# NVIDIA-Genomics-Research/racon-gpu

Hardware: AMD Instinct MI355X
Metric: Mbp polished/sec (whole node), ONT C.elegans, at 1/2/4/8 MI355X (higher is better)
Workload: dtype int16

## Files before the change

### src/hip/hip_polisher.cpp

```cpp
#include <hip/hip_runtime.h>

#include <atomic>
#include <chrono>
#include <memory>
#include <mutex>
#include <stdexcept>
#include <string>
#include <thread>
#include <tuple>
#include <utility>
#include <vector>

#include "core/polisher.hpp"
#include "hip/aligner_batch.hpp"
#include "hip/hip_common.hpp"
#include "hip/poa_batch.hpp"

namespace rga {

namespace {

struct BatchPools {
  std::mutex mutex;
  std::vector<std::pair<uint64_t, std::unique_ptr<hip::AlignerBatch>>> aligner;
// ... 424 lines not shown
    }
    const auto& bb = layers.front();
    auto w = createWindow(0, 0, tgs ? WindowType::kTGS : WindowType::kNGS,
                          std::get<0>(bb).data(),
                          static_cast<uint32_t>(std::get<0>(bb).size()),
                          std::get<1>(bb).data(),
                          static_cast<uint32_t>(std::get<1>(bb).size()));
    for (size_t i = 1; i < layers.size(); ++i) {
      const auto& l = layers[i];
      const std::string& q = std::get<1>(l);
      w->add_layer(std::get<0>(l).data(), static_cast<uint32_t>(std::get<0>(l).size()),
                   q.empty() ? nullptr : q.data(), static_cast<uint32_t>(q.size()),
                   std::get<2>(l), std::get<3>(l));
    }
    windows.push_back(std::move(w));
  }
  return windows;
}

std::vector<std::pair<std::string, bool>> poa_windows_gpu(
    const std::vector<std::vector<std::tuple<std::string, std::string, uint32_t, uint32_t>>>&
        window_layers,
    int8_t match, int8_t mismatch, int8_t gap, bool banded, bool trim, bool tgs,
    bool large_graphs, bool score_check) {
  std::vector<std::pair<std::string, bool>> out(window_layers.size());
  std::vector<std::shared_ptr<Window>> windows =
      windows_from_layers(window_layers, tgs, "poa_windows_gpu");

  hip::PoaBatch batch(0, 4ull << 30, match, mismatch, gap, banded, 200, large_graphs,
                      score_check);
  size_t begin = 0;
  std::vector<int64_t> slot_of(windows.size(), -1);
  auto flush = [&](size_t end) {
    std::vector<bool> status = batch.generate(trim);
    size_t k = 0;
    for (size_t i = begin; i < end; ++i) {
      if (slot_of[i] >= 0) {
        out[i] = {windows[i]->consensus(), status[k++]};
      }
    }
    batch.reset();
    begin = end;
  };
  size_t next_slot = 0;
  for (size_t i = 0; i < windows.size(); ++i) {
    if (windows[i]->num_layers() < 3) {
      auto bb = windows[i]->sequence(0);
      out[i] = {std::string(bb.first, bb.second), false};
      continue;
    }
    bool never_fits = false;
    if (batch.add_window(windows[i], &never_fits)) {
      slot_of[i] = static_cast<int64_t>(next_slot++);
      continue;
    }
    if (never_fits) {
      out[i] = {std::string(), false};
      continue;
    }
    flush(i);
    next_slot = 0;
    if (batch.add_window(windows[i], &never_fits)) {
      slot_of[i] = static_cast<int64_t>(next_slot++);
    } else {
      out[i] = {std::string(), false};
    }
  }
  flush(windows.size());
  return out;
}

std::vector<std::tuple<int32_t, std::vector<uint16_t>, std::vector<std::vector<uint16_t>>>>
poa_window_graph_gpu(const RawWindows& window_layers, int8_t match, int8_t mismatch, int8_t gap,
                     bool banded, bool large_graphs, bool score_check) {
  std::vector<std::shared_ptr<Window>> windows =
      windows_from_layers(window_layers, true, "poa_window_graph_gpu");
  hip::PoaBatch batch(0, 4ull << 30, match, mismatch, gap, banded, 200, large_graphs,
                      score_check);
  for (const auto& w : windows) {
    bool never_fits = false;
    if (w->num_layers() < 3 || !batch.add_window(w, &never_fits)) {
      throw std::runtime_error(
          "poa_window_graph_gpu: every window must run on the device, in one batch");
    }
  }
  std::vector<std::tuple<int32_t, std::vector<uint16_t>, std::vector<std::vector<uint16_t>>>> out(
      windows.size());
  if (windows.empty()) {
    return out;
  }
  (void)batch.generate(false);
  for (size_t i = 0; i < windows.size(); ++i) {
    const hip::PoaBatch::WindowGraph g = batch.read_graph(static_cast<uint32_t>(i));
    std::vector<std::vector<uint16_t>> edges(g.rank.size());
    for (size_t node = 0; node < edges.size(); ++node) {
      const uint16_t* row = g.out_edges.data() + node * hip::kPoaLimits.max_edges;
      edges[node].assign(row, row + std::min<uint32_t>(g.out_cnt[node], hip::kPoaLimits.max_edges));
    }
    out[i] = {g.status, g.rank, std::move(edges)};
  }
  return out;
// ... 109 lines not shown
```

### src/hip/hip_polisher_stub.cpp

```cpp
#include <cstdio>
#include <cstdlib>
#include <memory>
#include <string>
#include <tuple>
#include <utility>
#include <vector>

#include "core/polisher.hpp"
#include "hip/aligner_types.hpp"
#include "hip/comm.hpp"
#include "hip/poa_types.hpp"

namespace rga {

namespace comm {
Communicator::~Communicator() {}
void Communicator::init(int, int, const std::string&, int, bool) {
  fprintf(stderr, "[rga::comm] error: no HIP backend in this build!\n");
  exit(1);
}
void Communicator::finalize() {}
std::vector<std::string> Communicator::gather(const std::string&, int) { return {}; }
double Communicator::allreduce_max(double v) { return v; }
double Communicator::allreduce_sum(double v) { return v; }
void Communicator::barrier() {}
void Communicator::ctl_send(int, const void*, size_t) {}
void Communicator::ctl_recv(int, void*, size_t) {}
std::vector<std::string> Communicator::ctl_gather(const std::string&, int) { return {}; }
void Communicator::ctl_bcast(void*, size_t, int) {}
Communicator& world_comm() {
  static Communicator c;
  return c;
}
}

namespace hip {
int runtime_device_count() { return 0; }
void runtime_device_synchronize() {}
void release_batch_pools() {}
std::vector<std::pair<std::string, bool>> poa_windows_gpu(
    const std::vector<std::vector<std::tuple<std::string, std::string, uint32_t, uint32_t>>>&,
    int8_t, int8_t, int8_t, bool, bool, bool, bool, bool) {
  fprintf(stderr, "[rga::hip::poa_windows_gpu] error: no HIP backend in this build!\n");
  exit(1);
}
std::vector<std::tuple<int32_t, std::vector<uint16_t>, std::vector<std::vector<uint16_t>>>>
poa_window_graph_gpu(
    const std::vector<std::vector<std::tuple<std::string, std::string, uint32_t, uint32_t>>>&,
    int8_t, int8_t, int8_t, bool, bool, bool) {
  fprintf(stderr, "[rga::hip::poa_window_graph_gpu] error: no HIP backend in this build!\n");
  exit(1);
}
std::vector<std::tuple<std::string, int32_t, int32_t>> align_pairs(
    const std::vector<std::pair<std::string, std::string>>&, uint32_t, AlnBandPolicy,
    bool) {
  fprintf(stderr, "[rga::hip::align_pairs] error: no HIP backend in this build!\n");
  exit(1);
}
std::vector<std::tuple<std::vector<std::pair<uint32_t, uint32_t>>, int32_t, int32_t>>
breaking_points_pairs(const std::vector<std::pair<std::string, std::string>>&, uint32_t,
                      const std::vector<uint32_t>&, const std::vector<uint32_t>&, uint32_t,
                      AlnBandPolicy, bool) {
  fprintf(stderr, "[rga::hip::breaking_points_pairs] error: no HIP backend in this build!\n");
  exit(1);
}
}

std::unique_ptr<Polisher> createHipPolisher(std::unique_ptr<SequenceParser>,
                                            std::unique_ptr<OverlapParser>,
                                            std::unique_ptr<SequenceParser>, PolisherConfig) {
  fprintf(stderr,
          "[racon::createPolisher] error: HIP pipeline requested but this build "
// ... 6 lines not shown
```

### src/hip/poa_batch.cpp

```cpp
#include "hip/poa_batch.hpp"

#include <hip/hip_runtime.h>

#include <algorithm>
#include <chrono>
#include <cstring>
#include <stdexcept>
#include <type_traits>

#include "hip/hip_common.hpp"

namespace rga::hip {

namespace {

constexpr size_t kSeqArenaPerWindow = 96 * 1024;

constexpr PoaLimits L = kPoaLimits;
constexpr PoaLimits LL = kPoaLargeLimits;

constexpr size_t kLargeBudgetDivisor = 4;
constexpr size_t kLargeSlabCap = 2048;
constexpr size_t kLargePerWindow =
    poa_slab_bytes<true>() + LL.max_consensus * 3 + sizeof(PoaWindowDesc) + 1024;
// ... 112 lines not shown
    if (large_slabs_ > 1) {
      large_slabs_ /= 2;
    }
  }

  RGA_HIP_TRY(hipHostMalloc(reinterpret_cast<void**>(&h_seq_), seq_arena_cap_));
  RGA_HIP_TRY(hipHostMalloc(reinterpret_cast<void**>(&h_weight_), seq_arena_cap_));
  RGA_HIP_TRY(hipHostMalloc(reinterpret_cast<void**>(&h_layer_ends_), max_layers * 4));
  RGA_HIP_TRY(hipHostMalloc(reinterpret_cast<void**>(&h_layer_span_), max_layers * 4));
  RGA_HIP_TRY(hipHostMalloc(reinterpret_cast<void**>(&h_layer_index_), (num_slabs_ + 1) * 4));
  RGA_HIP_TRY(hipHostMalloc(reinterpret_cast<void**>(&h_desc_),
                            num_slabs_ * sizeof(PoaWindowDesc)));
  RGA_HIP_TRY(hipHostMalloc(reinterpret_cast<void**>(&h_consensus_),
                            static_cast<size_t>(num_slabs_) * L.max_consensus));
  RGA_HIP_TRY(hipHostMalloc(reinterpret_cast<void**>(&h_coverage_),
                            static_cast<size_t>(num_slabs_) * L.max_consensus * 2));
  RGA_HIP_TRY(hipHostMalloc(reinterpret_cast<void**>(&h_consensus_len_), num_slabs_ * 4));
  RGA_HIP_TRY(hipHostMalloc(reinterpret_cast<void**>(&h_status_), num_slabs_ * 4));

  lay_out(d_pool_);
  arena_.match = match_;
  arena_.mismatch = mismatch_;
  arena_.gap = gap_;
  arena_.band_width = banded ? 256 : 0;

  if (large_slabs_ != 0) {
    allocate_large_pool();
  }
}

void PoaBatch::allocate_large_pool() {
  large_arena_ = arena_;
  auto lay_out = [&](void* base) {
    size_t total = 0;
    auto carve = [&](auto*& p, size_t count) {
      p = reinterpret_cast<std::remove_reference_t<decltype(p)>>(
          reinterpret_cast<uintptr_t>(base) + total);
      total += (count * sizeof(*p) + 255) & ~size_t(255);
    };
    const size_t slabs = large_slabs_;
    carve(large_arena_.layer_ends_index, slabs + 1);
    carve(large_arena_.windows, slabs);
    for_each_poa_slab<true>(large_arena_.slabs,
                            [&](auto*& p, size_t count) { carve(p, slabs * count); });
    carve(large_arena_.timing, slabs * kPoaTimingSlots);
    carve(large_arena_.consensus, slabs * LL.max_consensus);
// ... 190 lines not shown
  std::vector<PoaWindowDesc> desc_sorted(nw0);
  std::vector<uint32_t> lidx_sorted(nw0);
  launch_slot_.assign(nw0, 0);
  for (uint32_t w = 0; w < nw0; ++w) {
    desc_sorted[w] = h_desc_[perm[w]];
    lidx_sorted[w] = h_layer_index_[perm[w]];
    launch_slot_[perm[w]] = w;
  }
  std::copy(desc_sorted.begin(), desc_sorted.end(), h_desc_);
  std::copy(lidx_sorted.begin(), lidx_sorted.end(), h_layer_index_);

  RGA_HIP_CHECK(hipSetDevice(device_));
  auto s = static_cast<hipStream_t>(stream_);
  auto d = [&](const void* dst, const void* src, size_t bytes) {
    RGA_HIP_CHECK(hipMemcpyAsync(const_cast<void*>(dst), src, bytes, hipMemcpyHostToDevice, s));
  };
  d(arena_.seq_data, h_seq_, seq_bytes_);
  d(arena_.weight_data, h_weight_, seq_bytes_);
  d(arena_.layer_ends, h_layer_ends_, num_layer_ends_ * 4);
  d(arena_.layer_spans, h_layer_span_, num_layer_ends_ * 4);
  d(arena_.layer_ends_index, h_layer_index_, windows_.size() * 4);
  d(arena_.windows, h_desc_, windows_.size() * sizeof(PoaWindowDesc));

  for (uint32_t begin = 0, end; begin < nw0; begin = end) {
    const PoaVariant v = variant_of[perm[begin]];
    for (end = begin + 1; end < nw0 && variant_of[perm[end]] == v; ++end) {
    }
    if (score_check_) {
      launch_poa_kernel_checked(arena_, begin, end - begin, v, stream_);
    } else {
      launch_poa_kernel(arena_, begin, end - begin, v, stream_);
    }
  }

  const size_t nw = windows_.size();
  RGA_HIP_CHECK(hipMemcpyAsync(h_consensus_, arena_.consensus,
                               nw * L.max_consensus, hipMemcpyDeviceToHost, s));
  RGA_HIP_CHECK(hipMemcpyAsync(h_coverage_, arena_.coverage,
                               nw * L.max_consensus * 2, hipMemcpyDeviceToHost, s));
  RGA_HIP_CHECK(hipMemcpyAsync(h_consensus_len_, arena_.consensus_len, nw * 4,
                               hipMemcpyDeviceToHost, s));
  RGA_HIP_CHECK(hipMemcpyAsync(h_status_, arena_.status, nw * 4, hipMemcpyDeviceToHost, s));
  auto t1 = clk::now();
  RGA_HIP_CHECK(hipStreamSynchronize(s));
  auto t2 = clk::now();

  large_completed_ = 0;
  large_slab_of_.assign(nw, -1);
  large_nodes_of_.assign(nw, 0);
  auto t_post = t2;
  if (large_slabs_ != 0) {
    const uint32_t ran = run_large_pass();
    t_post = clk::now();
    if (host_timing && ran != 0) {
      fprintf(stderr,
              "[rga::hip::PoaBatch] host timing: large-graph pass over %u window(s) %.1f ms\n",
              ran,
              std::chrono::duration_cast<std::chrono::microseconds>(t_post - t2).count() /
                  1000.0);
    }
  }

  if (getenv("RGA_POA_TIMING") != nullptr) {
    constexpr size_t kSlots = kPoaTimingSlots;
    std::vector<unsigned long long> t(nw * kSlots);
    RGA_HIP_CHECK(hipMemcpy(t.data(), arena_.timing, t.size() * sizeof(t[0]),
                            hipMemcpyDeviceToHost));
    unsigned long long sum[kSlots] = {0};
    std::vector<unsigned long long> totals(nw);
    for (size_t i = 0; i < nw; ++i) {
      for (size_t k = 0; k < kSlots; ++k) sum[k] += t[i * kSlots + k];
      totals[i] = t[i * kSlots + 6];
    }
    std::sort(totals.begin(), totals.end());
    fprintf(stderr,
            "[rga::hip::PoaBatch] timing (wall ticks, %zu windows): dp=%llu tb=%llu "
            "add=%llu topo=%llu rdesc=%llu cons=%llu total=%llu layers=%llu\n"
            "[rga::hip::PoaBatch] window total ticks: p50=%llu p90=%llu p99=%llu max=%llu\n",
            nw, sum[0], sum[1], sum[2], sum[3], sum[4], sum[5], sum[6], sum[7],
            totals[nw / 2], totals[nw * 9 / 10], totals[nw * 99 / 100], totals[nw - 1]);
  }

  score_refused_ = 0;
  for (size_t i = 0; i < nw; ++i) {
    const uint32_t orig = perm[i];
    auto& window = windows_[orig];
    if (h_status_[i] == kPoaScoreRange) {
      ++score_refused_;
    }
    if (h_status_[i] != kPoaOk || h_consensus_len_[i] == 0) {
      polished[orig] = false;
      continue;
    }
    std::string consensus(reinterpret_cast<char*>(h_consensus_ + i * L.max_consensus),
                          h_consensus_len_[i]);
    bool status = true;
    if (window->type() == WindowType::kTGS && trim) {
      const uint16_t* cov = h_coverage_ + i * L.max_consensus;
      uint32_t average = seqs_added_[orig] / 2;
      int32_t begin = 0, end = static_cast<int32_t>(consensus.size()) - 1;
      for (; begin < static_cast<int32_t>(consensus.size()); ++begin) {
        if (cov[begin] >= average) {
// ... 91 lines not shown
    for (uint32_t k = 0; k < n; ++k) {
      const uint32_t slot = todo[begin + k];
      h_status_[slot] = h_large_status_[k];
      h_consensus_len_[slot] = h_large_consensus_len_[k];
      std::memcpy(h_consensus_ + static_cast<size_t>(slot) * L.max_consensus,
                  h_large_consensus_ + static_cast<size_t>(k) * LL.max_consensus,
                  LL.max_consensus);
      std::memcpy(h_coverage_ + static_cast<size_t>(slot) * L.max_consensus,
                  h_large_coverage_ + static_cast<size_t>(k) * LL.max_consensus,
                  LL.max_consensus * 2);
      large_slab_of_[slot] = static_cast<int32_t>(k);
      large_nodes_of_[slot] = h_large_num_nodes_[k];
      large_slab_owner_[k] = slot;
    }

    if (timing) {
      constexpr size_t kSlots = kPoaTimingSlots;
      std::vector<unsigned long long> t(n * kSlots);
      RGA_HIP_CHECK(hipMemcpy(t.data(), large_arena_.timing, t.size() * sizeof(t[0]),
                              hipMemcpyDeviceToHost));
      unsigned long long sum[kSlots] = {0};
      unsigned long long longest = 0;
      for (size_t i = 0; i < n; ++i) {
        for (size_t k = 0; k < kSlots; ++k) sum[k] += t[i * kSlots + k];
        longest = std::max(longest, t[i * kSlots + 6]);
      }
      fprintf(stderr,
              "[rga::hip::PoaBatch] large-graph pass timing (wall ticks, %u windows): dp=%llu "
              "tb=%llu add=%llu topo=%llu rdesc=%llu cons=%llu total=%llu layers=%llu max=%llu\n",
              n, sum[0], sum[1], sum[2], sum[3], sum[4], sum[5], sum[6], sum[7], longest);
    }
  }
  return static_cast<uint32_t>(todo.size());
}

PoaBatch::WindowGraph PoaBatch::read_graph(uint32_t index) const {
  if (index >= launch_slot_.size() || launch_slot_.size() != windows_.size()) {
    throw std::runtime_error("[rga::hip::PoaBatch] read_graph: no such window in the last run");
  }
  RGA_HIP_CHECK(hipSetDevice(device_));
  WindowGraph g;
  g.status = h_status_[launch_slot_[index]];
  if (g.status != kPoaOk) {
    return g;
  }
  uint32_t n = 0;
  const PoaSlabs* slabs = &arena_.slabs;
// ... 20 lines not shown
    slab = static_cast<size_t>(index) * L.max_nodes;
  }
  static_assert(L.max_edges == LL.max_edges);
  g.rank.resize(n);
  g.out_cnt.resize(n);
  g.out_edges.resize(static_cast<size_t>(n) * L.max_edges);
  if (n != 0) {
    RGA_HIP_CHECK(hipMemcpy(g.rank.data(), slabs->rank + slab, n * sizeof(uint16_t),
                            hipMemcpyDeviceToHost));
    RGA_HIP_CHECK(hipMemcpy(g.out_cnt.data(), slabs->out_cnt + slab, n,
                            hipMemcpyDeviceToHost));
    RGA_HIP_CHECK(hipMemcpy(g.out_edges.data(), slabs->out_edges + slab * L.max_edges,
                            g.out_edges.size() * sizeof(uint16_t), hipMemcpyDeviceToHost));
  }
  return g;
}

void PoaBatch::reset() {
  launch_slot_.clear();
  large_slab_of_.clear();
  large_nodes_of_.clear();
  large_completed_ = 0;
  score_refused_ = 0;
  windows_.clear();
  seqs_added_.clear();
  pending_orders_.clear();
  packed_upto_ = 0;
  seq_bytes_ = 0;
  num_layer_ends_ = 0;
}

}
```

### src/hip/poa_batch.hpp

```cpp
#pragma once

#include <cstdint>
#include <memory>
#include <vector>

#include "core/window.hpp"
#include "hip/poa_types.hpp"

namespace rga::hip {

class PoaBatch {
 public:
  PoaBatch(int device, size_t mem_budget, int8_t match, int8_t mismatch, int8_t gap,
           bool banded, uint32_t max_depth, bool large_graphs = false,
           bool score_check = false);
  ~PoaBatch();

  PoaBatch(const PoaBatch&) = delete;
  PoaBatch& operator=(const PoaBatch&) = delete;

  bool add_window(const std::shared_ptr<Window>& window, bool* never_fits);

  void pack();

  uint32_t size() const { return static_cast<uint32_t>(windows_.size()); }
  uint32_t capacity() const { return num_slabs_; }

  static bool large_scores_fit(int8_t match, int8_t mismatch, int8_t gap, bool banded);
  uint32_t large_capacity() const { return large_slabs_; }
  uint32_t large_completed() const { return large_completed_; }

  static bool score_check_applies(int8_t match, int8_t mismatch, int8_t gap, bool banded,
                                  bool score_check);
  bool score_checked() const { return score_check_; }
  uint32_t score_refused() const { return score_refused_; }

  std::vector<bool> generate(bool trim);

  struct WindowGraph {
    int32_t status = kPoaNotRun;
    std::vector<uint16_t> rank;
    std::vector<uint8_t> out_cnt;
    std::vector<uint16_t> out_edges;
  };
  WindowGraph read_graph(uint32_t index) const;

  void reset();

 private:
  void allocate_arenas(bool banded);
  void allocate_large_pool();
  void release_all();
  uint32_t run_large_pass();

  int device_;
  void* stream_ = nullptr;

  uint32_t num_slabs_;
  size_t seq_arena_cap_;
  int8_t match_, mismatch_, gap_;
  uint32_t max_depth_;
  bool score_check_ = false;
  uint32_t score_refused_ = 0;

  uint8_t* h_seq_ = nullptr;
  uint8_t* h_weight_ = nullptr;
  uint32_t* h_layer_ends_ = nullptr;
  uint32_t* h_layer_span_ = nullptr;
  uint32_t* h_layer_index_ = nullptr;
  PoaWindowDesc* h_desc_ = nullptr;
  uint8_t* h_consensus_ = nullptr;
  uint16_t* h_coverage_ = nullptr;
  uint32_t* h_consensus_len_ = nullptr;
  int32_t* h_status_ = nullptr;

  void* d_pool_ = nullptr;
  PoaDeviceArena arena_{};

  size_t seq_bytes_ = 0;
  size_t num_layer_ends_ = 0;
  std::vector<std::shared_ptr<Window>> windows_;
  std::vector<uint32_t> seqs_added_;
  std::vector<std::vector<uint32_t>> pending_orders_;
  size_t packed_upto_ = 0;
  std::vector<uint32_t> launch_slot_;

// ... 18 lines not shown
```

### src/hip/poa_kernel.hip

```cpp
#include <hip/hip_runtime.h>

#include <cstdio>
#include <cstdlib>

#include "hip/poa_types.hpp"

namespace rga::hip {

namespace {

constexpr int kLanes = 64;
constexpr int32_t kNegInf = -(1 << 28);
#ifdef RGA_POA_LARGE_CLASS
constexpr bool kLarge = true;
#else
constexpr bool kLarge = false;
#endif
#ifdef RGA_POA_SCORE_CHECK
constexpr bool kChecked = true;
#else
constexpr bool kChecked = false;
#endif
constexpr PoaLimits kL = poa_limits(kLarge);
constexpr uint32_t kMaxW = kL.matrix_width;
// ... 855 lines not shown
      if (cbase + WB < kMaxW) {
        *reinterpret_cast<uint64_t*>(Mrow + cbase) = mvpack;
      } else {
        for (uint32_t w = 0; w < nown; ++w) {
          Mrow[cbase + w] = static_cast<uint8_t>(mvpack >> (8 * w));
        }
      }
    }
    if (len > base && len <= base + kLanes * WB) {
      const int owner = static_cast<int>((len - 1 - base) / WB);
      last_col_val = __builtin_amdgcn_readlane(h_sel, owner);
    }
  }

  wave_lds_sync();

  if ((is_end || (d.sub && r == d.rhi)) && last_col_val > best_score) {
    best_score = last_col_val;
    best_row = r + 1;
  }
}


constexpr uint32_t kTbDepth = 64;
static_assert(kTbDepth <= kLanes, "one lane per predicted move");

#define RGA_GLOBAL __attribute__((address_space(1)))
struct TracebackArrays {
  RGA_GLOBAL const uint8_t* moves;
  RGA_GLOBAL const uint64_t* row_desc;
  RGA_GLOBAL const uint16_t* rank;
  RGA_GLOBAL const uint16_t* in_edges;
  RGA_GLOBAL int32_t* aln_nodes;
};
using LdsU16 = __attribute__((address_space(3))) uint16_t;

__device__ __attribute__((noinline)) int32_t traceback_d(const TracebackArrays c, LdsU16* pred0,
                                                         uint32_t rlo, uint32_t best_row,
                                                         uint32_t len, int lane) {
  int32_t status = kPoaOk;
  for (uint32_t r = rlo + 1 + lane; r <= best_row; r += kLanes) {
    const uint32_t p = static_cast<uint32_t>((c.row_desc[r - 1] >> 32) & 0xffff);
    pred0[r] = static_cast<uint16_t>(p > rlo ? p : 0);
  }
  __syncthreads();

// ... 87 lines not shown
  static_assert(MAXW <= kMaxW, "ring width exceeds the slab matrix width");
  static_assert(MAXN <= kMaxN, "node cap exceeds the slab graph capacity");
  if (blockIdx.x >= num_windows) {
    return;
  }
  const uint32_t win = window_base + blockIdx.x;
  const int lane = threadIdx.x;
  const PoaWindowDesc desc = a.windows[win];

  __shared__ Shared<MAXW, MAXN> s;

  WindowCtx c;
  static_cast<PoaSlabs&>(c) = a.slabs;
  for_each_poa_slab<kLarge>(c, [slab = static_cast<size_t>(desc.scratch_idx)](auto*& p,
                                                                              size_t count) {
    p += slab * count;
  });

  unsigned long long* timing = a.timing + static_cast<size_t>(win) * kPoaTimingSlots;
  unsigned long long tick = TIMED ? wall_clock64() : 0;
  const unsigned long long t_start = tick;
  unsigned long long t_dp = 0, t_tb = 0, t_add = 0, t_topo = 0, t_rd = 0, t_cons = 0;
  unsigned long long layers_done = 0;
  auto lap = [&]() -> unsigned long long {
    if (!TIMED) {
      return 0;
    }
    unsigned long long now = wall_clock64();
    unsigned long long d = now - tick;
    tick = now;
    return d;
  };

  c.seq_base = a.seq_data + desc.seq_offset;
  c.weight_base = a.weight_data + desc.seq_offset;
  c.ends = a.layer_ends + a.layer_ends_index[win];
  c.spans = a.layer_spans + a.layer_ends_index[win];
  c.num_seqs = desc.num_seqs;
  c.MN = MAXN - 1;
  c.m = a.match;
  c.x = a.mismatch;
  c.g = a.gap;
  c.status = kPoaOk;

  init_backbone_d(c, s, lane);

// ... 7 lines not shown
    }
    if (len + 1 > MAXW) {
      c.status = kPoaWidthOverflow;
      break;
    }

    build_match_bits_d(s, seq, len, lane);

    const uint32_t n = c.num_nodes;
    LayerDp d;
    d.seq = seq;
    d.len = len;
    d.chunks = (len + kLanes - 1) / kLanes;
    const uint32_t span_word = c.spans[layer];
    d.sub = span_word != 0xFFFFFFFFu;
    d.rlo = d.sub ? c.rank[span_word >> 16] : 0;
    d.rhi = d.sub ? c.rank[span_word & 0xffffu] : n - 1;
    d.bw = a.band_width;
    d.banded = !CHECKED && (d.bw != 0) && (d.bw < len);
    d.slope16 = d.banded ? static_cast<uint32_t>((static_cast<uint64_t>(len) << 16) /
                                                 (d.rhi - d.rlo + 1))
                         : 0;

    int32_t best_score = kNegInf;
    uint32_t best_row = 0;
    uint32_t score_low = 0;
    (void)lap();

    for (uint32_t rblk = d.rlo & ~(kLanes - 1); rblk <= d.rhi; rblk += kLanes) {
      if (rblk + lane < n) {
        s.u.dp.rd_block[lane] = c.row_desc[rblk + lane];
        s.u.dp.rd2_block[lane] = c.row_desc2[rblk + lane];
      }
      wave_lds_sync();
      const uint32_t rlim = min(d.rhi + 1, rblk + kLanes);
      for (uint32_t r = max(rblk, d.rlo); r < rlim; ++r) {
        dp_row<CHECKED, WB, MAXW>(c, s, d, r, s.u.dp.rd_block[r - rblk],
                                  s.u.dp.rd2_block[r - rblk], lane, best_score, best_row,
                                  score_low);
      }
      wave_lds_sync();
    }

    t_dp += lap();
    ++layers_done;

    int lane_g = lane;
    asm volatile("" : "+v"(lane_g));

    if (CHECKED && score_low != 0) {
      c.status = kPoaScoreRange;
    }

    if (!CHECKED || c.status == kPoaOk) {
      c.status = traceback_d({(RGA_GLOBAL const uint8_t*)c.moves,
                              (RGA_GLOBAL const uint64_t*)c.row_desc,
                              (RGA_GLOBAL const uint16_t*)c.rank,
                              (RGA_GLOBAL const uint16_t*)c.in_edges,
                              (RGA_GLOBAL int32_t*)c.aln_nodes},
// ... 27 lines not shown
    t_rd += lap();
  }

  if (lane == 0) {
    uint8_t* out = a.consensus + static_cast<size_t>(win) * kL.max_consensus;
    uint16_t* cov = a.coverage + static_cast<size_t>(win) * kL.max_consensus;
    int32_t clen = -1;
    (void)lap();
    if (c.status == kPoaOk) {
      clen = consensus_d(c, s, out, cov, kL.max_consensus);
    }
    t_cons = lap();
    a.consensus_len[win] = clen < 0 ? 0 : static_cast<uint32_t>(clen);
    a.status[win] = c.status;
    a.num_nodes[win] = c.num_nodes;
    if (TIMED) {
      timing[0] = t_dp;
      timing[1] = t_tb;
      timing[2] = t_add;
      timing[3] = t_topo;
      timing[4] = t_rd;
      timing[5] = t_cons;
      timing[6] = wall_clock64() - t_start;
      timing[7] = layers_done;
    }
  }
}

#ifdef RGA_POA_SCORE_CHECK
#define RGA_POA_LAUNCH(name) name##_checked
#else
#define RGA_POA_LAUNCH(name) name
#endif

#ifdef RGA_POA_LARGE_CLASS
template <bool TIMED>
void launch_large(const PoaDeviceArena& arena, uint32_t window_base, uint32_t num_windows,
                  hipStream_t stream) {
  constexpr PoaVariantParams p = kPoaLargeVariant;
  hipLaunchKernelGGL((poa_window_kernel<TIMED, kChecked, p.cols_per_lane, p.ring_width,
                                        p.node_cap, p.min_waves>),
                     dim3(num_windows), dim3(kLanes), 0, stream, arena, window_base,
                     num_windows);
}

}

// ... 64 lines not shown
```

### src/hip/poa_types.hpp

```cpp
#pragma once

#include <cstddef>
#include <cstdint>
#include <initializer_list>

namespace rga::hip {

struct PoaLimits {
  uint32_t max_nodes = 2047;
  uint32_t max_edges = 48;
  uint32_t max_ring = 4;
  uint32_t matrix_width = 1024;
  uint32_t max_consensus = 2048;
};
inline constexpr PoaLimits kPoaLimits{};

inline constexpr PoaLimits kPoaLargeLimits{4095, 48, 4, 1024, 2048};
constexpr PoaLimits poa_limits(bool large) { return large ? kPoaLargeLimits : kPoaLimits; }
static_assert(kPoaLargeLimits.max_edges == kPoaLimits.max_edges &&
                  kPoaLargeLimits.max_ring == kPoaLimits.max_ring &&
                  kPoaLargeLimits.matrix_width == kPoaLimits.matrix_width &&
                  kPoaLargeLimits.max_consensus == kPoaLimits.max_consensus,
              "the classes differ in max_nodes alone: they share inputs and outputs");

// ... 13 lines not shown

constexpr int32_t poa_abs(int32_t v) { return v < 0 ? -v : v; }
constexpr int32_t poa_max(int32_t a, int32_t b) { return a > b ? a : b; }

constexpr bool poa_scores_fit_worst_case(const PoaLimits& l, int32_t m, int32_t x, int32_t g,
                                         bool banded) {
  const int32_t worst = static_cast<int32_t>(l.max_nodes + l.matrix_width) *
                        poa_max(poa_abs(m), poa_max(poa_abs(x), poa_abs(g)));
  return worst <= -(banded ? kPoaScoreFloorBanded : kPoaScoreFloor);
}

constexpr bool poa_score_check_static(int32_t m, int32_t x, int32_t g, uint32_t matrix_width) {
  return g < 0 && poa_max(poa_max(m, x), 0) * static_cast<int32_t>(matrix_width - 1) <=
                      -kPoaScoreFloor;
}

constexpr bool poa_score_row_refused(int32_t h0, uint32_t len, int32_t g) {
  return h0 + static_cast<int32_t>(len) * g < kPoaScoreFloor;
}
static_assert(poa_score_check_static(27, -20, -13, 1024) &&
              !poa_score_check_static(28, -20, -13, 1024) &&
              !poa_score_check_static(3, -5, 0, 1024));
static_assert(!poa_score_row_refused(-14000, 500, -28) && poa_score_row_refused(-14500, 500, -29));

enum PoaVariant : uint32_t {
  kPoaNarrow = 0,
  kPoaMid = 1,
  kPoaFull = 2,
  kPoaBandedMid = 3,
  kPoaBandedFull = 4,
  kPoaNumVariants
};

struct PoaVariantParams {
  uint32_t cols_per_lane;
  uint32_t ring_width;
  uint32_t node_cap;
  uint32_t min_waves;
};

inline constexpr PoaVariantParams kPoaLargeVariant = {8, kPoaLargeLimits.matrix_width,
                                                      kPoaLargeLimits.max_nodes + 1, 2};
static_assert(5 * kPoaLargeVariant.node_cap * (4 * kPoaLargeVariant.min_waves) <= 160 * 1024,
              "the large variant's Kahn side must leave min_waves waves per SIMD resident");

inline constexpr PoaVariantParams kPoaVariants[kPoaNumVariants] = {
// ... 60 lines not shown
  X(int32_t, aln_nodes, 2 * L.matrix_width + N)  \
  X(int32_t, aln_seq, 2 * L.matrix_width + N)    \
  X(int16_t, matrix, (N + 1) * L.matrix_width)   \
  X(uint8_t, moves, (N + 1) * L.matrix_width)    \
  X(uint64_t, row_desc, N)                       \
  X(uint64_t, row_desc2, N)

struct PoaSlabs {
#define RGA_X(T, name, count) T* name;
  RGA_POA_SLAB_ARRAYS(RGA_X)
#undef RGA_X
};

template <bool LARGE = false, class F>
constexpr void for_each_poa_slab(PoaSlabs& s, F&& f) {
  constexpr PoaLimits L = poa_limits(LARGE);
  constexpr size_t N = L.max_nodes;
#define RGA_X(T, name, count) f(s.name, static_cast<size_t>(count));
  RGA_POA_SLAB_ARRAYS(RGA_X)
#undef RGA_X
}

constexpr size_t kPoaTimingSlots = 8;

template <bool LARGE = false>
constexpr size_t poa_slab_bytes() {
  PoaSlabs s{};
  size_t b = kPoaTimingSlots * sizeof(unsigned long long);
  for_each_poa_slab<LARGE>(s, [&b](auto* p, size_t count) { b += count * sizeof(*p); });
  return b;
}
static_assert(poa_slab_bytes() == 7200396, "slab layout changed: batch sizes move with it");
static_assert(poa_slab_bytes<true>() == 14384780,
              "large slab layout changed: the large pool's size moves with it");

struct PoaDeviceArena {
  const uint8_t* seq_data;
  const uint8_t* weight_data;
  const uint32_t* layer_ends;
  const uint32_t* layer_spans;
  const uint32_t* layer_ends_index;
  const PoaWindowDesc* windows;

  PoaSlabs slabs;

  unsigned long long* timing;

  uint8_t* consensus;
  uint16_t* coverage;
  uint32_t* consensus_len;
  int32_t* status;
  uint32_t* num_nodes;

  int8_t match, mismatch, gap;
  uint32_t band_width;
};

void launch_poa_kernel(const PoaDeviceArena& arena, uint32_t window_base,
                       uint32_t num_windows, PoaVariant variant, void* stream);

void launch_poa_kernel_large(const PoaDeviceArena& arena, uint32_t window_base,
                             uint32_t num_windows, void* stream);

void launch_poa_kernel_checked(const PoaDeviceArena& arena, uint32_t window_base,
                               uint32_t num_windows, PoaVariant variant, void* stream);
void launch_poa_kernel_large_checked(const PoaDeviceArena& arena, uint32_t window_base,
                                     uint32_t num_windows, void* stream);

}
```

### src/py/module.cpp

```cpp
#include <pybind11/pybind11.h>
#include <pybind11/stl.h>

#include <memory>
#include <optional>
#include <stdexcept>
#include <string>
#include <utility>
#include <vector>

#include "align/pairwise.hpp"
#include "align/poa.hpp"
#include "core/polisher.hpp"
#include "core/sequence.hpp"
#include "hip/aligner_types.hpp"
#include "hip/comm.hpp"

namespace rga::hip {
int runtime_device_count();
void runtime_device_synchronize();
void release_batch_pools();
std::vector<std::tuple<std::string, int32_t, int32_t>> align_pairs(
    const std::vector<std::pair<std::string, std::string>>& pairs, uint32_t band_width,
    AlnBandPolicy policy, bool wide_pass);
std::vector<std::tuple<std::vector<std::pair<uint32_t, uint32_t>>, int32_t, int32_t>>
breaking_points_pairs(const std::vector<std::pair<std::string, std::string>>& pairs,
                      uint32_t window_length, const std::vector<uint32_t>& t_begins,
                      const std::vector<uint32_t>& q_begins, uint32_t band_width,
                      AlnBandPolicy policy, bool wide_pass);
std::vector<std::pair<std::string, bool>> poa_windows_gpu(
    const std::vector<std::vector<std::tuple<std::string, std::string, uint32_t, uint32_t>>>&
        window_layers,
    int8_t match, int8_t mismatch, int8_t gap, bool banded, bool trim, bool tgs,
    bool large_graphs, bool score_check);
std::vector<std::tuple<int32_t, std::vector<uint16_t>, std::vector<std::vector<uint16_t>>>>
poa_window_graph_gpu(
    const std::vector<std::vector<std::tuple<std::string, std::string, uint32_t, uint32_t>>>&
        window_layers,
    int8_t match, int8_t mismatch, int8_t gap, bool banded, bool large_graphs, bool score_check);
}

namespace py = pybind11;

namespace {

std::vector<std::pair<std::string, std::string>> polish(
    const std::string& sequences_path, const std::string& overlaps_path,
    const std::string& target_path, bool fragment_correction, uint32_t window_length,
    double quality_threshold, double error_threshold, bool trim, int8_t match, int8_t mismatch,
    int8_t gap, uint32_t threads, uint32_t poa_batches, bool banded_poa, uint32_t aligner_batches,
    uint32_t aligner_band_width, bool include_unpolished, bool aligner_adaptive_band,
    bool aligner_wide_band, bool poa_large_graphs, bool poa_score_check) {
  rga::PolisherConfig config;
  config.type = fragment_correction ? rga::PolisherType::kF : rga::PolisherType::kC;
  config.window_length = window_length;
  config.quality_threshold = quality_threshold;
  config.error_threshold = error_threshold;
  config.trim = trim;
  config.match = match;
  config.mismatch = mismatch;
  config.gap = gap;
  config.num_threads = threads;
// ... 276 lines not shown
        py::arg("band_policy") = "diagonal", py::kw_only(), py::arg("wide_pass") = false,
        "GPU Myers aligner in breaking-point mode on raw (query, target) pairs whose "
        "target / query start at t_begins[k] / q_begins[k] -> ([(t, q), ...], "
        "edit_distance, status)");
  m.def("breaking_points_from_cigar", &breaking_points_from_cigar_py, py::arg("cigar"),
        py::arg("window_length"), py::arg("t_begin"), py::arg("t_end"), py::arg("q_begin"),
        "Per-window (target, query) breaking points of a CIGAR over [t_begin, t_end): "
        "first match and last match + 1 of every window that has a match.");
  m.def("reverse_complement", &reverse_complement, py::arg("sequence"));
  m.def("poa_windows_cpu", &poa_windows_cpu, py::arg("windows"), py::arg("match") = 3,
        py::arg("mismatch") = -5, py::arg("gap") = -4, py::arg("trim") = true,
        py::arg("tgs") = true);
  m.def("poa_window_score_bounds", &poa_window_score_bounds, py::arg("windows"),
        py::arg("match") = 3, py::arg("mismatch") = -5, py::arg("gap") = -4,
        "CPU model of the HIP POA engine's score check: per window (check_min, true_min, "
        "true_max) over the DP matrices of all its layers in the CPU engine. check_min is the "
        "smallest H[row][0] + len * gap, which the device compares with -28000; true_min and "
        "true_max are the smallest and largest cells.");
  m.def("poa_window_node_counts", &poa_window_node_counts, py::arg("windows"),
        py::arg("match") = 3, py::arg("mismatch") = -5, py::arg("gap") = -4);
  m.def("poa_windows_gpu", [](const std::vector<std::vector<
                                  std::tuple<std::string, std::string, uint32_t, uint32_t>>>& w,
                              int8_t match, int8_t mismatch, int8_t gap, bool banded,
                              bool trim, bool tgs, bool large_graphs, bool score_check) {
    py::gil_scoped_release release;
    return rga::hip::poa_windows_gpu(w, match, mismatch, gap, banded, trim, tgs, large_graphs,
                                     score_check);
  }, py::arg("windows"), py::arg("match") = 3, py::arg("mismatch") = -5,
     py::arg("gap") = -4, py::arg("banded") = false, py::arg("trim") = true,
     py::arg("tgs") = true, py::arg("large_graphs") = false, py::arg("score_check") = false);
  m.def("poa_window_graph_gpu",
        [](const std::vector<
               std::vector<std::tuple<std::string, std::string, uint32_t, uint32_t>>>& w,
           int8_t match, int8_t mismatch, int8_t gap, bool banded, bool large_graphs,
           bool score_check) {
          py::gil_scoped_release release;
          return rga::hip::poa_window_graph_gpu(w, match, mismatch, gap, banded, large_graphs,
                                                score_check);
        },
        py::arg("windows"), py::arg("match") = 3, py::arg("mismatch") = -5, py::arg("gap") = -4,
        py::arg("banded") = false, py::arg("large_graphs") = false,
        py::arg("score_check") = false,
        "Test entry: the windows through the GPU POA kernel in one batch, then per window "
        "(status, rank per node, out-edge targets per node) read back from its slab; the "
        "lists are empty unless status is 0. large_graphs: with the large-graph pass, whose "
        "windows are read back from their large slabs. score_check: with the per-window "
        "score check; a refused window has status 7.");
  m.def("poa_consensus", &poa_consensus, py::arg("sequences"),
        py::arg("qualities") = std::vector<std::string>(), py::arg("match") = 5,
        py::arg("mismatch") = -4, py::arg("gap") = -8);
  m.attr("__version__") = "1.0.0";
}
```

Baseline: 11.59.

## Add packed-int16 fast path for single-predecessor POA DP rows

Adds a specialized DP row routine for rows whose node has exactly one predecessor, an ACGT base, an in-ring predecessor, and a layer length up to 512 in the unbanded, unchecked, narrow kernel. It computes eight columns per lane with packed 16-bit vector ops, a wave max-scan for the left-gap recurrence, and packed move bytes, replacing the general per-row routine. The path is on by default, gated by an env var and a score-range fit check. It also packs lean/total row counts into the timing slot. Risks are an extra branch per row and correctness depending on int16 headroom.

```diff
diff --git a/src/hip/hip_polisher.cpp b/src/hip/hip_polisher.cpp
--- a/src/hip/hip_polisher.cpp
+++ b/src/hip/hip_polisher.cpp
@@ -470,13 +470,14 @@
     const std::vector<std::vector<std::tuple<std::string, std::string, uint32_t, uint32_t>>>&
         window_layers,
     int8_t match, int8_t mismatch, int8_t gap, bool banded, bool trim, bool tgs,
-    bool large_graphs, bool score_check) {
+    bool large_graphs, bool score_check, bool lean_rows) {
   std::vector<std::pair<std::string, bool>> out(window_layers.size());
   std::vector<std::shared_ptr<Window>> windows =
       windows_from_layers(window_layers, tgs, "poa_windows_gpu");
 
   hip::PoaBatch batch(0, 4ull << 30, match, mismatch, gap, banded, 200, large_graphs,
                       score_check);
+  batch.set_lean_rows(lean_rows);
   size_t begin = 0;
   std::vector<int64_t> slot_of(windows.size(), -1);
   auto flush = [&](size_t end) {
@@ -488,6 +489,7 @@
       }
     }
     batch.reset();
+    batch.set_lean_rows(lean_rows);
     begin = end;
   };
   size_t next_slot = 0;
@@ -520,11 +522,12 @@
 
 std::vector<std::tuple<int32_t, std::vector<uint16_t>, std::vector<std::vector<uint16_t>>>>
 poa_window_graph_gpu(const RawWindows& window_layers, int8_t match, int8_t mismatch, int8_t gap,
-                     bool banded, bool large_graphs, bool score_check) {
+                     bool banded, bool large_graphs, bool score_check, bool lean_rows) {
   std::vector<std::shared_ptr<Window>> windows =
       windows_from_layers(window_layers, true, "poa_window_graph_gpu");
   hip::PoaBatch batch(0, 4ull << 30, match, mismatch, gap, banded, 200, large_graphs,
                       score_check);
+  batch.set_lean_rows(lean_rows);
   for (const auto& w : windows) {
     bool never_fits = false;
     if (w->num_layers() < 3 || !batch.add_window(w, &never_fits)) {
diff --git a/src/hip/hip_polisher_stub.cpp b/src/hip/hip_polisher_stub.cpp
--- a/src/hip/hip_polisher_stub.cpp
+++ b/src/hip/hip_polisher_stub.cpp
@@ -40,14 +40,14 @@
 void release_batch_pools() {}
 std::vector<std::pair<std::string, bool>> poa_windows_gpu(
     const std::vector<std::vector<std::tuple<std::string, std::string, uint32_t, uint32_t>>>&,
-    int8_t, int8_t, int8_t, bool, bool, bool, bool, bool) {
+    int8_t, int8_t, int8_t, bool, bool, bool, bool, bool, bool) {
   fprintf(stderr, "[rga::hip::poa_windows_gpu] error: no HIP backend in this build!\n");
   exit(1);
 }
 std::vector<std::tuple<int32_t, std::vector<uint16_t>, std::vector<std::vector<uint16_t>>>>
 poa_window_graph_gpu(
     const std::vector<std::vector<std::tuple<std::string, std::string, uint32_t, uint32_t>>>&,
-    int8_t, int8_t, int8_t, bool, bool, bool) {
+    int8_t, int8_t, int8_t, bool, bool, bool, bool) {
   fprintf(stderr, "[rga::hip::poa_window_graph_gpu] error: no HIP backend in this build!\n");
   exit(1);
 }
diff --git a/src/hip/poa_batch.cpp b/src/hip/poa_batch.cpp
--- a/src/hip/poa_batch.cpp
+++ b/src/hip/poa_batch.cpp
@@ -158,6 +158,7 @@
   arena_.match = match_;
   arena_.mismatch = mismatch_;
   arena_.gap = gap_;
+  arena_.lean_rows = 0;
   arena_.band_width = banded ? 256 : 0;
 
   if (large_slabs_ != 0) {
@@ -394,6 +395,13 @@
   d(arena_.layer_ends_index, h_layer_index_, windows_.size() * 4);
   d(arena_.windows, h_desc_, windows_.size() * sizeof(PoaWindowDesc));
 
+  static const bool lean_env = [] {
+    const char* e = getenv("RGA_POA_LEAN_ROWS");
+    return e == nullptr || atoi(e) != 0;
+  }();
+  arena_.lean_rows =
+      lean_rows_ && lean_env && poa_lean_rows_fit(match_, mismatch_, gap_) ? 1 : 0;
+
   for (uint32_t begin = 0, end; begin < nw0; begin = end) {
     const PoaVariant v = variant_of[perm[begin]];
     for (end = begin + 1; end < nw0 && variant_of[perm[end]] == v; ++end) {
@@ -440,16 +448,22 @@
                             hipMemcpyDeviceToHost));
     unsigned long long sum[kSlots] = {0};
     std::vector<unsigned long long> totals(nw);
+    unsigned long long rows = 0, lean = 0;
     for (size_t i = 0; i < nw; ++i) {
-      for (size_t k = 0; k < kSlots; ++k) sum[k] += t[i * kSlots + k];
+      for (size_t k = 0; k < kSlots - 1; ++k) sum[k] += t[i * kSlots + k];
+      sum[7] += poa_count_layers(t[i * kSlots + 7]);
+      lean += poa_count_lean_rows(t[i * kSlots + 7]);
+      rows += poa_count_rows(t[i * kSlots + 7]);
       totals[i] = t[i * kSlots + 6];
     }
     std::sort(totals.begin(), totals.end());
     fprintf(stderr,
             "[rga::hip::PoaBatch] timing (wall ticks, %zu windows): dp=%llu tb=%llu "
-            "add=%llu topo=%llu rdesc=%llu cons=%llu total=%llu layers=%llu\n"
+            "add=%llu topo=%llu rdesc=%llu cons=%llu total=%llu layers=%llu rows=%llu "
+            "lean_rows=%llu (%.1f%%)\n"
             "[rga::hip::PoaBatch] window total ticks: p50=%llu p90=%llu p99=%llu max=%llu\n",
-            nw, sum[0], sum[1], sum[2], sum[3], sum[4], sum[5], sum[6], sum[7],
+            nw, sum[0], sum[1], sum[2], sum[3], sum[4], sum[5], sum[6], sum[7], rows, lean,
+            rows != 0 ? 100.0 * static_cast<double>(lean) / static_cast<double>(rows) : 0.0,
             totals[nw / 2], totals[nw * 9 / 10], totals[nw * 99 / 100], totals[nw - 1]);
   }
 
@@ -587,7 +601,8 @@
       unsigned long long sum[kSlots] = {0};
       unsigned long long longest = 0;
       for (size_t i = 0; i < n; ++i) {
-        for (size_t k = 0; k < kSlots; ++k) sum[k] += t[i * kSlots + k];
+        for (size_t k = 0; k < kSlots - 1; ++k) sum[k] += t[i * kSlots + k];
+        sum[7] += poa_count_layers(t[i * kSlots + 7]);
         longest = std::max(longest, t[i * kSlots + 6]);
       }
       fprintf(stderr,
@@ -654,6 +669,7 @@
   large_nodes_of_.clear();
   large_completed_ = 0;
   score_refused_ = 0;
+  lean_rows_ = true;
   windows_.clear();
   seqs_added_.clear();
   pending_orders_.clear();
diff --git a/src/hip/poa_batch.hpp b/src/hip/poa_batch.hpp
--- a/src/hip/poa_batch.hpp
+++ b/src/hip/poa_batch.hpp
@@ -35,6 +35,9 @@
   bool score_checked() const { return score_check_; }
   uint32_t score_refused() const { return score_refused_; }
 
+  void set_lean_rows(bool on) { lean_rows_ = on; }
+  bool lean_rows() const { return lean_rows_; }
+
   std::vector<bool> generate(bool trim);
 
   struct WindowGraph {
@@ -62,6 +65,7 @@
   uint32_t max_depth_;
   bool score_check_ = false;
   uint32_t score_refused_ = 0;
+  bool lean_rows_ = true;
 
   uint8_t* h_seq_ = nullptr;
   uint8_t* h_weight_ = nullptr;
diff --git a/src/hip/poa_kernel.hip b/src/hip/poa_kernel.hip
--- a/src/hip/poa_kernel.hip
+++ b/src/hip/poa_kernel.hip
@@ -901,6 +901,174 @@
 }
 
 
+using pk16 = short __attribute__((ext_vector_type(2)));
+using pku16 = unsigned short __attribute__((ext_vector_type(2)));
+
+__device__ __forceinline__ pk16 pk_from(uint32_t w) { return __builtin_bit_cast(pk16, w); }
+__device__ __forceinline__ uint32_t pk_bits(pk16 v) { return __builtin_bit_cast(uint32_t, v); }
+__device__ __forceinline__ pk16 pk_splat(int32_t v) {
+  return pk16{static_cast<short>(v), static_cast<short>(v)};
+}
+__device__ __forceinline__ pk16 pk_max(pk16 a, pk16 b) { return __builtin_elementwise_max(a, b); }
+__device__ __forceinline__ pk16 pk_lo(pk16 a) { return __builtin_shufflevector(a, a, 0, 0); }
+__device__ __forceinline__ pk16 pk_hi(pk16 a) { return __builtin_shufflevector(a, a, 1, 1); }
+__device__ __forceinline__ pk16 pk_next(pk16 a, pk16 b) {
+  return pk_from(__builtin_amdgcn_alignbit(pk_bits(b), pk_bits(a), 16));
+}
+__device__ __forceinline__ uint32_t pk_differ(pk16 a, pk16 b) {
+  const uint32_t x = pk_bits(a) ^ pk_bits(b);
+  uint32_t r;
+  asm("v_pk_min_u16 %0, %1, %2" : "=v"(r) : "v"(x), "s"(0x00010001u));
+  return r;
+}
+
+__device__ __forceinline__ int32_t poa_code_uniform(uint32_t letter) {
+  const uint32_t idx = letter - 'A';
+  if (idx > 19u || ((0x80045u >> idx) & 1u) == 0) {
+    return -1;
+  }
+  const uint32_t t = (letter >> 1) & 3u;
+  return static_cast<int32_t>(t ^ (t >> 1));
+}
+static_assert((('A' >> 1) & 3) == 0 && (('C' >> 1) & 3) == 1 && (('G' >> 1) & 3) == 3 &&
+              (('T' >> 1) & 3) == 2 && 'C' - 'A' == 2 && 'G' - 'A' == 6 && 'T' - 'A' == 19);
+
+template <uint32_t MAXW, class SH>
+__device__ __forceinline__ void dp_row_lean(const WindowCtx c, SH& s, const LayerDp& d,
+                                            uint32_t r, uint32_t rd_hi, int32_t code, int lane_id,
+                                            int32_t& best_score, uint32_t& best_row) {
+  constexpr uint32_t WB = 8;
+  int lane = lane_id;
+  asm volatile("" : "+v"(lane));
+  static_assert(kLanes * WB + 1 <= MAXW, "column cbase + 8 of lane 63 is inside the ring row");
+  static_assert(kLanes * WB == kPoaLeanMaxLen);
+  static_assert(kLanes * WB < kMaxW, "a lane's eight move bytes never reach the column-0 slot");
+  const uint32_t len = d.len;
+  const uint32_t pred0 = rd_hi & 0xffffu;
+  const bool is_end = ((rd_hi >> 16) & kRdEnd) != 0;
+  const bool store_row = ((rd_hi >> 16) & kRdStore) != 0;
+  int16_t* Hrow = c.matrix + static_cast<size_t>(r + 1) * kMaxW;
+  uint8_t* Mrow = c.moves + static_cast<size_t>(r + 1) * kMaxW;
+  int16_t* ring_row = s.u.dp.ring[(r + 1) % kRing];
+  const int16_t* pred_row = s.u.dp.ring[pred0 % kRing];
+
+  const uint32_t cbase = static_cast<uint32_t>(lane) * WB;
+  const int4 pvec = *reinterpret_cast<const int4*>(&pred_row[cbase]);
+  const uint32_t pv8 = static_cast<uint16_t>(pred_row[cbase + WB]);
+  const uint32_t mb = reinterpret_cast<const uint8_t*>(s.u.dp.match[code])[lane];
+
+  const int32_t h0 =
+      static_cast<int16_t>(__builtin_amdgcn_readfirstlane(pvec.x) & 0xffff) + c.g;
+
+  const pk16 P[4] = {pk_from(pvec.x), pk_from(pvec.y), pk_from(pvec.z), pk_from(pvec.w)};
+  const pk16 N[4] = {pk_next(P[0], P[1]), pk_next(P[1], P[2]), pk_next(P[2], P[3]),
+                     pk_next(P[3], pk_from(pv8))};
+  const pk16 gg = pk_splat(c.g);
+  const pku16 xx = __builtin_bit_cast(pku16, pk_splat(c.x));
+  const pku16 mx = __builtin_bit_cast(pku16, pk_splat(c.m - c.x));
+  const uint32_t spread = mb * 0x8001u;
+  const int32_t jg0 = static_cast<int32_t>(cbase + 1) * c.g;
+  const pk16 jg01 = pk16{static_cast<short>(jg0), static_cast<short>(jg0 + c.g)};
+  pk16 V[4], JG[4];
+  uint32_t up[4];
+#pragma unroll
+  for (uint32_t q = 0; q < 4; ++q) {
+    const pku16 bit = __builtin_bit_cast(pku16, (spread >> (2 * q)) & 0x00010001u);
+    const pk16 subst = __builtin_bit_cast(pk16, static_cast<pku16>(bit * mx + xx));
+    const pk16 bd = P[q] + subst;
+    const pk16 bu = N[q] + gg;
+    V[q] = pk_max(bd, bu);
+    up[q] = pk_differ(V[q], bd);
+    JG[q] = jg01 + pk_splat(static_cast<int32_t>(2 * q) * c.g);
+  }
+
+  pk16 R[4];
+#pragma unroll
+  for (uint32_t q = 0; q < 4; ++q) {
+    const pk16 u = V[q] - JG[q];
+    R[q] = pk_max(u, pk_lo(u));
+    if (q != 0) {
+      R[q] = pk_max(R[q], pk_hi(R[q - 1]));
+    }
+  }
+  const int32_t run = static_cast<int32_t>(pk_bits(R[3])) >> 16;
+  const int32_t incl = wave_scan_max(run);
+  int32_t excl = __builtin_amdgcn_update_dpp(kNegInf, incl, 0x138, 0xf, 0xf, false);
+  excl = max(excl, h0);
+  const pk16 ex = pk_from(__builtin_amdgcn_perm(0u, static_cast<uint32_t>(excl), 0x01000100u));
+
+  const pk16 floor2 = pk_splat(kPoaScoreFloor);
+  pk16 H[4], HC[4];
+  uint32_t mv[4];
+#pragma unroll
+  for (uint32_t q = 0; q < 4; ++q) {
+    H[q] = pk_max(R[q], ex) + JG[q];
+    HC[q] = pk_max(H[q], floor2);
+    const uint32_t left = pk_differ(H[q], V[q]);
+    static_assert(kMvDiag == 0 && kMvUp == 1 && kMvLeft == 2);
+    mv[q] = __builtin_bit_cast(
+        uint32_t, __builtin_elementwise_max(__builtin_bit_cast(pku16, up[q]),
+                                            __builtin_bit_cast(pku16, left + left)));
+  }
+  uint64_t mvpack =
+      static_cast<uint64_t>(__builtin_amdgcn_perm(mv[1], mv[0], 0x06040200u)) |
+      (static_cast<uint64_t>(__builtin_amdgcn_perm(mv[3], mv[2], 0x06040200u)) << 32);
+
+  const uint32_t shifted = static_cast<uint32_t>(__builtin_amdgcn_update_dpp(
+      static_cast<int32_t>(static_cast<uint32_t>(h0) << 16), static_cast<int32_t>(pk_bits(HC[3])),
+      0x138, 0xf, 0xf, false));
+  if (cbase < len) {
+    int4 vec;
+    vec.x = static_cast<int32_t>(__builtin_amdgcn_alignbit(pk_bits(HC[0]), shifted, 16));
+    vec.y = static_cast<int32_t>(pk_bits(pk_next(HC[0], HC[1])));
+    vec.z = static_cast<int32_t>(pk_bits(pk_next(HC[1], HC[2])));
+    vec.w = static_cast<int32_t>(pk_bits(pk_next(HC[2], HC[3])));
+    *reinterpret_cast<int4*>(&ring_row[cbase]) = vec;
+    if (store_row) {
+      *reinterpret_cast<int4*>(Hrow + cbase) = vec;
+    }
+    const uint32_t nown = min(WB, len - cbase);
+    if (nown < WB) {
+      mvpack &= (1ull << (8 * nown)) - 1;
+    }
+    *reinterpret_cast<uint64_t*>(Mrow + cbase) = mvpack;
+  }
+  if (lane == 0) {
+    Mrow[kMaxW - 1] = kMvUp;
+  }
+  if ((len & (WB - 1)) == 0) {
+    const uint32_t t16 =
+        static_cast<uint32_t>(__builtin_amdgcn_readlane(static_cast<int32_t>(pk_bits(HC[3])),
+                                                        static_cast<int>(len / WB) - 1)) >> 16;
+    if (lane == 0) {
+      ring_row[len] = static_cast<int16_t>(t16);
+      if (store_row) {
+        Hrow[len] = static_cast<int16_t>(t16);
+      }
+    }
+  }
+
+  wave_lds_sync();
+
+  if (is_end || (d.sub && r == d.rhi)) {
+    const int owner = static_cast<int>((len - 1) / WB);
+    const uint32_t w = (len - 1) & (WB - 1);
+    const uint32_t s0 = __builtin_amdgcn_readlane(static_cast<int32_t>(pk_bits(H[0])), owner);
+    const uint32_t s1 = __builtin_amdgcn_readlane(static_cast<int32_t>(pk_bits(H[1])), owner);
+    const uint32_t s2 = __builtin_amdgcn_readlane(static_cast<int32_t>(pk_bits(H[2])), owner);
+    const uint32_t s3 = __builtin_amdgcn_readlane(static_cast<int32_t>(pk_bits(H[3])), owner);
+    const uint32_t pair = w < 2 ? s0 : w < 4 ? s1 : w < 6 ? s2 : s3;
+    const int32_t last_col_val =
+        (w & 1) != 0 ? static_cast<int32_t>(pair) >> 16
+                     : static_cast<int32_t>(static_cast<int16_t>(pair & 0xffffu));
+    if (last_col_val > best_score) {
+      best_score = last_col_val;
+      best_row = r + 1;
+    }
+  }
+}
+
+
 constexpr uint32_t kTbDepth = 64;
 static_assert(kTbDepth <= kLanes, "one lane per predicted move");
 
@@ -1034,6 +1202,8 @@
   const unsigned long long t_start = tick;
   unsigned long long t_dp = 0, t_tb = 0, t_add = 0, t_topo = 0, t_rd = 0, t_cons = 0;
   unsigned long long layers_done = 0;
+  uint32_t rows_done = 0, rows_lean = 0;
+  constexpr bool kLeanKernel = WB == 8 && !kLarge && !CHECKED;
   auto lap = [&]() -> unsigned long long {
     if (!TIMED) {
       return 0;
@@ -1087,6 +1257,8 @@
                                                  (d.rhi - d.rlo + 1))
                          : 0;
 
+    const bool lean_layer = kLeanKernel && a.lean_rows != 0 && !d.banded && len <= kPoaLeanMaxLen;
+
     int32_t best_score = kNegInf;
     uint32_t best_row = 0;
     uint32_t score_low = 0;
@@ -1100,6 +1272,28 @@
       wave_lds_sync();
       const uint32_t rlim = min(d.rhi + 1, rblk + kLanes);
       for (uint32_t r = max(rblk, d.rlo); r < rlim; ++r) {
+        if constexpr (kLeanKernel) {
+          if (lean_layer) {
+            const uint64_t rdv = s.u.dp.rd_block[r - rblk];
+            const uint32_t rd_lo = __builtin_amdgcn_readfirstlane(static_cast<uint32_t>(rdv));
+            const uint32_t rd_hi =
+                __builtin_amdgcn_readfirstlane(static_cast<uint32_t>(rdv >> 32));
+            const uint32_t pred0 = rd_hi & 0xffffu;
+            const int32_t code = poa_code_uniform(rd_lo & 0xffu);
+            if (((rd_lo >> 8) & 0xffu) == 1 && code >= 0 && r + 1 - pred0 < kRing &&
+                (!d.sub || pred0 > d.rlo)) {
+              dp_row_lean<MAXW>(c, s, d, r, rd_hi, code, lane, best_score, best_row);
+              if (TIMED) {
+                ++rows_lean;
+                ++rows_done;
+              }
+              continue;
+            }
+          }
+        }
+        if (TIMED) {
+          ++rows_done;
+        }
         dp_row<CHECKED, WB, MAXW>(c, s, d, r, s.u.dp.rd_block[r - rblk],
                                   s.u.dp.rd2_block[r - rblk], lane, best_score, best_row,
                                   score_low);
@@ -1173,7 +1367,7 @@
       timing[4] = t_rd;
       timing[5] = t_cons;
       timing[6] = wall_clock64() - t_start;
-      timing[7] = layers_done;
+      timing[7] = poa_pack_counts(layers_done, rows_lean, rows_done);
     }
   }
 }
diff --git a/src/hip/poa_types.hpp b/src/hip/poa_types.hpp
--- a/src/hip/poa_types.hpp
+++ b/src/hip/poa_types.hpp
@@ -59,6 +59,16 @@
               !poa_score_check_static(28, -20, -13, 1024) &&
               !poa_score_check_static(3, -5, 0, 1024));
 static_assert(!poa_score_row_refused(-14000, 500, -28) && poa_score_row_refused(-14500, 500, -29));
+
+inline constexpr uint32_t kPoaLeanMaxLen = 512;
+constexpr bool poa_lean_rows_fit(int32_t m, int32_t x, int32_t g) {
+  return g < 0 && -kPoaScoreFloor + poa_max(poa_abs(m), poa_max(poa_abs(x), poa_abs(g))) +
+                          static_cast<int32_t>(kPoaLeanMaxLen) * poa_abs(g) <=
+                      32767;
+}
+static_assert(poa_lean_rows_fit(3, -5, -4) && poa_lean_rows_fit(5, -4, -8) &&
+              poa_lean_rows_fit(3, -8, -4) && poa_lean_rows_fit(9, -9, -9) &&
+              !poa_lean_rows_fit(3, -5, 0) && !poa_lean_rows_fit(3, -5, -10));
 
 enum PoaVariant : uint32_t {
   kPoaNarrow = 0,
@@ -165,6 +175,15 @@
 }
 
 constexpr size_t kPoaTimingSlots = 8;
+constexpr unsigned long long poa_pack_counts(unsigned long long layers, unsigned long long lean,
+                                             unsigned long long rows) {
+  return layers | (lean << 16) | (rows << 40);
+}
+constexpr unsigned long long poa_count_layers(unsigned long long w) { return w & 0xffffu; }
+constexpr unsigned long long poa_count_lean_rows(unsigned long long w) {
+  return (w >> 16) & 0xffffffu;
+}
+constexpr unsigned long long poa_count_rows(unsigned long long w) { return w >> 40; }
 
 template <bool LARGE = false>
 constexpr size_t poa_slab_bytes() {
@@ -196,6 +215,7 @@
   uint32_t* num_nodes;
 
   int8_t match, mismatch, gap;
+  uint8_t lean_rows;
   uint32_t band_width;
 };
 
diff --git a/src/py/module.cpp b/src/py/module.cpp
--- a/src/py/module.cpp
+++ b/src/py/module.cpp
@@ -31,12 +31,13 @@
     const std::vector<std::vector<std::tuple<std::string, std::string, uint32_t, uint32_t>>>&
         window_layers,
     int8_t match, int8_t mismatch, int8_t gap, bool banded, bool trim, bool tgs,
-    bool large_graphs, bool score_check);
+    bool large_graphs, bool score_check, bool lean_rows);
 std::vector<std::tuple<int32_t, std::vector<uint16_t>, std::vector<std::vector<uint16_t>>>>
 poa_window_graph_gpu(
     const std::vector<std::vector<std::tuple<std::string, std::string, uint32_t, uint32_t>>>&
         window_layers,
-    int8_t match, int8_t mismatch, int8_t gap, bool banded, bool large_graphs, bool score_check);
+    int8_t match, int8_t mismatch, int8_t gap, bool banded, bool large_graphs, bool score_check,
+    bool lean_rows);
 }
 
 namespace py = pybind11;
@@ -359,30 +360,33 @@
   m.def("poa_windows_gpu", [](const std::vector<std::vector<
                                   std::tuple<std::string, std::string, uint32_t, uint32_t>>>& w,
                               int8_t match, int8_t mismatch, int8_t gap, bool banded,
-                              bool trim, bool tgs, bool large_graphs, bool score_check) {
+                              bool trim, bool tgs, bool large_graphs, bool score_check,
+                              bool lean_rows) {
     py::gil_scoped_release release;
     return rga::hip::poa_windows_gpu(w, match, mismatch, gap, banded, trim, tgs, large_graphs,
-                                     score_check);
+                                     score_check, lean_rows);
   }, py::arg("windows"), py::arg("match") = 3, py::arg("mismatch") = -5,
      py::arg("gap") = -4, py::arg("banded") = false, py::arg("trim") = true,
-     py::arg("tgs") = true, py::arg("large_graphs") = false, py::arg("score_check") = false);
+     py::arg("tgs") = true, py::arg("large_graphs") = false, py::arg("score_check") = false,
+     py::arg("lean_rows") = true);
   m.def("poa_window_graph_gpu",
         [](const std::vector<
                std::vector<std::tuple<std::string, std::string, uint32_t, uint32_t>>>& w,
            int8_t match, int8_t mismatch, int8_t gap, bool banded, bool large_graphs,
-           bool score_check) {
+           bool score_check, bool lean_rows) {
           py::gil_scoped_release release;
           return rga::hip::poa_window_graph_gpu(w, match, mismatch, gap, banded, large_graphs,
-                                                score_check);
+                                                score_check, lean_rows);
         },
         py::arg("windows"), py::arg("match") = 3, py::arg("mismatch") = -5, py::arg("gap") = -4,
         py::arg("banded") = false, py::arg("large_graphs") = false,
-        py::arg("score_check") = false,
+        py::arg("score_check") = false, py::arg("lean_rows") = true,
         "Test entry: the windows through the GPU POA kernel in one batch, then per window "
         "(status, rank per node, out-edge targets per node) read back from its slab; the "
         "lists are empty unless status is 0. large_graphs: with the large-graph pass, whose "
         "windows are read back from their large slabs. score_check: with the per-window "
-        "score check; a refused window has status 7.");
+        "score check; a refused window has status 7. lean_rows=False: every DP row through the "
+        "general row (poa_windows_gpu takes the same switch).");
   m.def("poa_consensus", &poa_consensus, py::arg("sequences"),
         py::arg("qualities") = std::vector<std::string>(), py::arg("match") = 5,
         py::arg("mismatch") = -4, py::arg("gap") = -8);
```

Result: faster. 13.64 (median of 6 runs) (+17.7%).
